# hztools/go-sdr

Hardware: AMD Instinct MI355X
Metric: Msamples/s: u8->c64->Shift->FIR-decimate chain @1 GPU; 4-ch Beamform @1/2/4 GPU (higher is better)
Workload: dtype u8 x int32 fixed-point taps (int8 MFMA digit planes, exact) -> c64(f32), NCO phase 64-bit fixed point

## Files before the change

go-sdr_amd/csrc/hz_firmm2.h:

```cpp
#pragma once
#include <type_traits>

#include "hz_firmm.h"
#include "hz_firmm2_plan.h"

namespace hz {
namespace mm2 {

using mm::v16i;
using mm::v4i;

using mm::find_le;
using mm::task_window;

struct KernArgs {
    const void *in;
    float2 *out;
    const float2 *hist;
    float2 *new_hist;
    const uint8_t *rhist;
    uint8_t *new_rhist;
    const float2 *taps;
    size_t n_in;
    Geom G;
// ... 33 lines not shown
        return make_float2(__fmaf_rn(v.x, cr, -(v.y * ci)), __fmaf_rn(v.x, ci, v.y * cr));
    };
#pragma unroll
    for (int b = 0; b < NB; b++) {
        double zc = cc0, zs = cs0;
#pragma unroll
        for (int q = 0; q < 4; q++) {
            y[4 * b + q] = mul32(y[4 * b + q], zc, zs);
            if (q < 3) {
                const double nc = __fma_rn(zc, e_c, -(zs * e_s)), ns = __fma_rn(zc, e_s, zs * e_c);
                zc = nc;
                zs = ns;
            }
        }
        if (b + 1 < NB) {
            const double nc = __fma_rn(cc0, b_c, -(cs0 * b_s)), ns = __fma_rn(cc0, b_s, cs0 * b_c);
            cc0 = nc;
            cs0 = ns;
        }
    }
}

typedef float v2f __attribute__((ext_vector_type(2)));
__device__ __forceinline__ v2f pk_turn(v2f cs0, v2f wxy, v2f wzw) {
    v2f t;
    asm("v_pk_mul_f32 %0, %1, %2 op_sel:[1,1] op_sel_hi:[1,0] neg_lo:[0,1]" : "=v"(t) : "v"(cs0), "v"(wzw));
    asm("v_pk_fma_f32 %0, %1, %2, %0 op_sel_hi:[0,1,1]" : "+v"(t) : "v"(cs0), "v"(wzw));
    asm("v_pk_fma_f32 %0, %1, %2, %0 op_sel:[1,1,0] op_sel_hi:[1,0,1] neg_lo:[0,1,0]" : "+v"(t) : "v"(cs0), "v"(wxy));
    asm("v_pk_fma_f32 %0, %1, %2, %0 op_sel_hi:[0,1,1]" : "+v"(t) : "v"(cs0), "v"(wxy));
    return t;
}
__device__ __forceinline__ v2f pk_cmul(v2f y, v2f f) {
    v2f u, r;
    asm("v_pk_mul_f32 %0, %1, %2 op_sel:[1,1] op_sel_hi:[1,0] neg_lo:[0,1]" : "=v"(u) : "v"(y), "v"(f));
    asm("v_pk_fma_f32 %0, %1, %2, %3 op_sel_hi:[0,1,1]" : "=v"(r) : "v"(y), "v"(f), "v"(u));
    return r;
}

template <int FMT, int D, int NG = 0, int EXP = 0, int UG = 0>
__global__ __launch_bounds__(kThreads) void fir_mm2_kernel(
    const void *__restrict__ in, float2 *__restrict__ out, const float2 *__restrict__ hist,
    float2 *__restrict__ new_hist, const uint8_t *__restrict__ rhist, uint8_t *__restrict__ new_rhist,
    const float2 *__restrict__ taps, size_t n_in, Geom G, Plan L, EwProgram P, Fix F, Batch B,
    unsigned long long *stamps = nullptr) {
    extern __shared__ __attribute__((aligned(16))) uint8_t mm_lds[];
    constexpr int TB = tile_bytes(D), PPT = TB / 16, GS = PPT / 2, NB = blocks_for(D);
    constexpr int kPassOut = pass_out(D);
    constexpr bool STRAIGHT = NG > 0 && UG == 0;
    constexpr int KU = NG > 0 ? ((pass_tiles(D) - 1 + NG) * PPT + 63) / 64 : kU;
    constexpr bool kWhole = NG > 0 && ((pass_tiles(D) - 1 + NG) * PPT) % 64 == 0;
    constexpr bool kPlane = STRAIGHT && D == 8 && (EXP & (1 << 29)) != 0;
    static_assert(!kPlane || (EXP & (256 | 524288 | (1 << 23) | (1 << 27) | (1 << 28))) == 0, "not with the pair loop's experiments");
    static_assert(!kPlane || plane_form(D, NG * GS, 0), "the host sizes the LDS by plane_form");
    constexpr int TS = tile_stride(D, kPlane);
    const int tid = threadIdx.x, wave = __builtin_amdgcn_readfirstlane(tid >> 6), l = tid & 63;
    const int wb = blockIdx.x;
    const int n = l & 31, h = l >> 5;
    const size_t tab_lds = table_lds(G.ne), slot_sz = slot_bytes(D, G.ks, kPlane);
    uint8_t *const tabp = mm_lds;
    unsigned *const ctr = reinterpret_cast<unsigned *>(mm_lds + 2 * tab_lds);
    uint8_t *const slot = mm_lds + 2 * tab_lds + kCtlBytes + (size_t)wave * slot_sz;
    const int64_t n_bytes = 2 * (int64_t)n_in;
    const uint8_t *src = (const uint8_t *)in;
    const int pieces = (int)(image_bytes(D, G.ks) / 16);
    const int nbuf = B.nbuf;
    const uint32_t rcp = B.rcp;
    const int64_t nb = (int64_t)B.nb;
    auto buf_of = [&](uint32_t pass) -> int { return nbuf > 1 ? (int)__umulhi(pass, rcp) : 0; };
    auto vin_of = [&](int j) -> uint64_t { return j == 0 ? (uint64_t)(uintptr_t)src : B.vin[j]; };
    auto vout_of = [&](int j) -> uint64_t { return j == 0 ? (uint64_t)(uintptr_t)out : B.vout[j]; };
    typedef const v4i __attribute__((address_space(1))) *gload_p;
    constexpr bool kStampShare = kPlane && (EXP & 64) != 0;
    static_assert(!kStampShare || (8 * 16 * 8 * kWaves <= 8192 && 2 * slot_bytes(D, NG * GS, true) >= task_bytes(D, 1025)), "the shared areas fit");
    constexpr int kStampRows = (EXP & (1 << 24)) != 0 ? 16 : 4;
    int stamp_pass = 0;
    [[maybe_unused]] unsigned long long *const lstamp =
        reinterpret_cast<unsigned long long *>(mm_lds + lds_bytes(D, G.ks, G.ne, G.ntaps, kPlane) - (kStampShare ? task_bytes(D, G.ntaps) : 0)) +
        (size_t)wave * (8 * kStampRows);
    if constexpr ((EXP & 64) != 0) {
        for (int i = l; i < 8 * kStampRows; i += 64) lstamp[i] = 0;
    }
    auto stamp = [&](int k) {
        if constexpr ((EXP & 64) != 0) {
            if (l == 0 && stamp_pass < kStampRows)
                lstamp[(k == 0 || k == 7 || (k >= 8 && k < 16) ? 0 : stamp_pass) * 8 + (k & 7)] = __builtin_amdgcn_s_memrealtime();
        }
    };
    stamp(0);
    [[maybe_unused]] unsigned long long clk0 = 0, rt0 = 0;
    if constexpr ((EXP & 64) != 0) clk0 = __builtin_amdgcn_s_memtime(), rt0 = __builtin_amdgcn_s_memrealtime();
    if constexpr ((EXP & 32) != 0) __builtin_amdgcn_s_setprio(1);
    const Run run0 = L.run[0];
    {
        const uint64_t a0 = (uint64_t)(uintptr_t)in, a1 = (uint64_t)n_in, a2 = (uint64_t)(uintptr_t)run0.tab;
        asm volatile("" ::"s"(a0), "s"(a1), "s"(a2), "s"(G.w0), "s"(G.ks), "s"(G.ne), "s"(G.e0), "s"(G.ntaps), "s"(G.off), "s"(L.n),
                     "s"(L.n_pass), "s"(L.grid), "s"(L.n_task), "s"(L.pass_first[0]), "s"(L.pass_end[0]), "s"(L.pass_first[1]),
                     "s"(L.pass_end[1]), "s"(run0.m_lo), "s"(run0.m_hi), "s"(nbuf), "s"(rcp), "s"(nb));
    }

    const uint32_t NP = (uint32_t)L.n_pass;
    const uint32_t per = NP / (uint32_t)L.grid, rem = NP - per * (uint32_t)L.grid;
    const uint32_t pb0 = (uint32_t)wb * per + min((uint32_t)wb, rem), pb1 = pb0 + per + ((uint32_t)wb < rem ? 1u : 0u);

    auto pass_p0 = [&](uint32_t pass) { return 2 * ((int64_t)D * ((int64_t)pass * kPassOut) - G.w0); };
    auto inside = [&](uint32_t pass) {
        const int64_t p0 = pass_p0(pass), lo = (int64_t)buf_of(pass) * nb;
        return p0 >= lo && p0 + 16 * (int64_t)pieces <= lo + nb;
    };
    auto issue = [&](v4i(&x)[KU], uint32_t pass) {
        const gload_p p = (gload_p)(vin_of(buf_of(pass)) + (uint64_t)pass_p0(pass));
        const gload_p pl = p + l;
#pragma unroll
        for (int u = 0; u < KU; u++) {
            x[u] = v4i{0, 0, 0, 0};
            if constexpr ((EXP & 1) != 0) continue;
            if constexpr (kWhole) x[u] = __builtin_nontemporal_load(pl + 64 * u);
            else x[u] = __builtin_nontemporal_load(p + min(l + u * 64, pieces - 1));
        }
    };
    v4i x[KU];
    bool pre_issued = false;
    if (wave < kWaves / 2) {
        const uint32_t p = pb0 + (uint32_t)wave;
        if (pb0 >= (uint32_t)L.pass_first[0] && p < min(pb1, (uint32_t)L.pass_end[0]) && inside(p)) {
            issue(x, p);
            pre_issued = true;
        }
    }
    using RWT = typename Raw<FMT>::t;
    uint32_t fix_m0 = 0;
    int fix_cnt = 0;
    auto task_xs = [&](const Geom &G) {
        return reinterpret_cast<float2 *>(mm_lds + 2 * table_lds(G.ne) + kCtlBytes + (kStampShare ? 0 : (size_t)kWaves * slot_bytes(D, G.ks, kPlane)));
    };
    auto tasks_front_cold = [&](int round, const void *in, const float2 *hist, float2 *new_hist, const uint8_t *rhist, uint8_t *new_rhist,
                                const float2 *taps, size_t n_in, const Geom &G, const Plan &L, const EwProgram &P, const Fix &F, const Batch &B) {
        auto vbase = [&](int64_t pu) -> const RWT * {
            const void *sb = in;
            for (int i = 1; i < B.nbuf; i++)
                if (2 * pu >= (int64_t)i * (int64_t)B.nb) sb = (const void *)(uintptr_t)B.vin[i];
            return (const RWT *)sb;
        };
        float2 *const xs = task_xs(G);
        float2 *const tl = xs + (G.ntaps + D * (kFixOut - 1));
        const int ftask = (L.grid - 1 - wb) + round * L.grid;
        if (ftask < L.n_task) {
            const int ct = tid;
            const int k = find_le(F.task_first, F.n, ftask);
            fix_m0 = F.m_a[k] + (uint32_t)(ftask - F.task_first[k]) * kFixOut;
            fix_cnt = (int)min((uint32_t)kFixOut, F.m_b[k] - fix_m0);
            if (round == 0)
                for (int q = ct; q < G.ntaps; q += 256) tl[q] = taps[q];
            const int64_t p_lo = (int64_t)D * fix_m0 - (G.ntaps - 1);
            const int n_s = G.ntaps + D * (fix_cnt - 1);
            const NcoWin tw = task_window(P, p_lo, p_lo + n_s - 1);
#pragma unroll 1
            for (int i0 = ct; i0 < n_s; i0 += 5 * 256) {
                constexpr int W = 5;
                float2 v[W];
#pragma unroll
                for (int u = 0; u < W; u++) {
                    const int64_t pu = p_lo + i0 + u * 256;
                    v[u] = Raw<FMT>::cvt((i0 + u * 256 < n_s && pu >= 0) ? vbase(pu)[pu] : RWT{});
                }
                ew_apply_n<W, 2>(P, v, (uint64_t)(p_lo + i0), tw, (uint64_t)256);
#pragma unroll
                for (int u = 0; u < W; u++) {
                    const int idx = i0 + u * 256;
                    const int64_t pu = p_lo + idx;
                    if (idx < n_s)
                        xs[idx] = pu >= 0 ? v[u] : ((hist && pu + (int64_t)G.off >= 0) ? hist[pu + (int64_t)G.off] : make_float2(0.f, 0.f));
                }
            }
        }
    };
    auto history_tasks_cold = [&](const void *in0, const float2 *hist, float2 *new_hist, const uint8_t *rhist, uint8_t *new_rhist, size_t n_in,
                                  const Geom &G, const Plan &L, const EwProgram &P, const Batch &B) {
        const void *const in = B.nbuf > 1 ? (const void *)(uintptr_t)B.vin[B.nbuf - 1] : in0;
        const int n_hist_tasks = new_hist ? (int)((G.off + kHistPer - 1) / kHistPer) : 0;
        for (int j = wb + L.grid * wave; j < n_hist_tasks; j += (kWaves / 2) * L.grid) {
            const unsigned idx = (unsigned)j * kHistPer + l;
            const int64_t h_lo = (int64_t)n_in - (int64_t)G.off + (int64_t)j * kHistPer;
            const NcoWin tw = task_window(P, h_lo, h_lo + kHistPer - 1);
            if (idx < G.off) {
                const int64_t p = (int64_t)n_in - (int64_t)G.off + idx;
                new_hist[idx] = mm::ordered_sample<FMT, 2>(in, P, p, hist, G.off, tw);
// ... 13 lines not shown
    auto tasks_front = [&](int round) {
        if (wave >= kWaves / 2) return;
        if ((L.grid - 1 - wb) + round * L.grid >= L.n_task) return;
        if constexpr ((EXP & 4096) != 0) {
            tasks_front_cold(round, in, hist, new_hist, rhist, new_rhist, taps, n_in, G, L, P, F, B);
        } else {
            HZ_COLD_ARGS;
            tasks_front_cold(round, in, hist, new_hist, rhist, new_rhist, taps, n_in, G, L, P, F, B);
        }
    };
    auto tasks_back_cold = [&](float2 *out0, const Geom &G, const Batch &B) {
        float2 *const xs = task_xs(G);
        float2 *const tl = xs + (G.ntaps + D * (kFixOut - 1));
        const int ct = tid;
        const int o = ct >> 4, sl = ct & 15;
        double ar = 0.0, ai = 0.0;
        if (o < fix_cnt) {
            const float2 *xo = xs + D * o + (G.ntaps - 1);
#pragma unroll 4
            for (int kk = sl; kk < G.ntaps; kk += 16) {
                const float2 hk = tl[kk], x = xo[-kk];
                const double xr = x.x, xi = x.y, hr = hk.x, hi = hk.y;
                ar = __fma_rn(xr, hr, ar);
                ar = __fma_rn(-xi, hi, ar);
                ai = __fma_rn(xr, hi, ai);
                ai = __fma_rn(xi, hr, ai);
            }
        }
#pragma unroll
        for (int d = 1; d < 16; d <<= 1) {
            ar += __shfl_xor(ar, d);
            ai += __shfl_xor(ai, d);
        }
        if (o < fix_cnt && sl == 0) {
            float2 *ob = out0;
            for (int i = 1; i < B.nbuf; i++)
                if (fix_m0 + o >= (uint32_t)i * B.out_each) ob = (float2 *)(uintptr_t)B.vout[i];
            ob[fix_m0 + o] = make_float2((float)ar, (float)ai);
        }
        fix_cnt = 0;
    };
    auto tasks_back = [&]() {
        if (wave >= kWaves / 2 || fix_cnt == 0) return;
        if constexpr ((EXP & 4096) != 0) {
            tasks_back_cold(out, G, B);
        } else {
            HZ_COLD_ARGS;
            tasks_back_cold(out, G, B);
        }
    };
    stamp(9);
    auto put = [&](int q, v4i v) {
        if constexpr (FMT == HZSDR_FMT_U8) v ^= (int)0x80808080;
        *reinterpret_cast<v4i *>(slot + TS * (q / PPT) + 16 * (q % PPT)) = v;
    };
    auto vm_clear = [&]() {
        if constexpr ((EXP & 128) == 0) __builtin_amdgcn_s_waitcnt(0x0F70);
    };
    auto land = [&](v4i(&x)[KU], bool flipped = false) {
        uint8_t *lp = slot + TS * (l / PPT) + 16 * (l % PPT);
        if constexpr (FMT == HZSDR_FMT_U8 && STRAIGHT && (EXP & 262144) != 0 && (EXP & (1 << 25)) != 0 && (EXP & 32768) == 0) {
            if (!flipped) {
#pragma unroll
                for (int u = 0; u < KU; u++) {
                    x[u] ^= (int)0x80808080;
                    asm volatile("" : "+v"(x[u]));
                }
            }
        }
#pragma unroll
        for (int u = 0; u < KU; u++)
            if (kWhole || l + u * 64 < pieces) {
                if constexpr (FMT == HZSDR_FMT_U8 && (EXP & 32768) == 0) {
                    if constexpr (STRAIGHT && (EXP & 262144) != 0 && (EXP & (1 << 25)) != 0) {
                    } else if constexpr (STRAIGHT && (EXP & 262144) != 0) {
                        if (!flipped) x[u] ^= (int)0x80808080;
                    } else {
                        x[u] ^= (int)0x80808080;
                    }
                }
                *reinterpret_cast<v4i *>(lp + u * (64 / PPT) * TS) = x[u];
            }
        if constexpr (FMT == HZSDR_FMT_U8 && (EXP & 32768) != 0) {
#pragma unroll
            for (int u = 0; u < KU; u++)
                if (kWhole || l + u * 64 < pieces) {
                    unsigned long long *q8 = reinterpret_cast<unsigned long long *>(lp + u * (64 / PPT) * TS);
                    (void)__hip_atomic_fetch_xor(q8, 0x8080808080808080ull, __ATOMIC_RELAXED, __HIP_MEMORY_SCOPE_WAVEFRONT);
                    (void)__hip_atomic_fetch_xor(q8 + 1, 0x8080808080808080ull, __ATOMIC_RELAXED, __HIP_MEMORY_SCOPE_WAVEFRONT);
                }
        }
        __builtin_amdgcn_fence(__ATOMIC_RELEASE, "wavefront");
        __builtin_amdgcn_wave_barrier();
    };
    auto land_edge_cold = [&](uint32_t pass, const uint8_t *src, const uint8_t *rhist, int64_t n_bytes, const Geom &G, const Plan &L, const Batch &B) {
        const int64_t p0 = 2 * ((int64_t)D * ((int64_t)pass * kPassOut) - G.w0);
        const int pieces = (int)(image_bytes(D, G.ks) / 16);
#pragma unroll 1
        for (int q = l; q < pieces; q += 64) {
            const int64_t p = p0 + (int64_t)q * 16;
            v4i v{0, 0, 0, 0};
            if (p >= 0 && p + 16 <= n_bytes) {
                uint64_t sb = (uint64_t)(uintptr_t)src;
                for (int i = 1; i < B.nbuf; i++)
                    if (p >= (int64_t)i * (int64_t)B.nb) sb = B.vin[i];
                v = *(const v4i __attribute__((address_space(1))) *)(sb + (uint64_t)p);
            } else if (p < 0 && L.cont && p + 2 * (int64_t)G.off >= 0) {
                v = *reinterpret_cast<const v4i *>(rhist + (p + 2 * (int64_t)G.off));
            } else if (p + 16 > 0 && p < n_bytes) {
                uint64_t w0 = 0, w1 = 0;
#pragma unroll 1
                for (int e = 0; e < 16; e++)
                    if (p + e >= 0 && p + e < n_bytes) {
                        const uint64_t bb = src[p + e];
                        if (e < 8) w0 |= bb << (8 * e);
                        else w1 |= bb << (8 * (e - 8));
                    }
                v = v4i{(int)(uint32_t)w0, (int)(uint32_t)(w0 >> 32), (int)(uint32_t)w1, (int)(uint32_t)(w1 >> 32)};
            }
            put(q, v);
        }
        __builtin_amdgcn_fence(__ATOMIC_RELEASE, "wavefront");
        __builtin_amdgcn_wave_barrier();
    };
    auto land_edge = [&](uint32_t pass) {
        if constexpr ((EXP & 4096) != 0) {
            land_edge_cold(pass, src, rhist, n_bytes, G, L, B);
        } else {
            HZ_COLD_ARGS;
            land_edge_cold(pass, (const uint8_t *)in, rhist, 2 * (int64_t)n_in, G, L, B);
        }
    };

    const int i_row = 4 * ((n >> 2) & 1) + (n >> 3);
    const int a_base = 64 * ((D / 8) * i_row - h + G.e0) + 16 * (n & 3);
    const int f_stride = G.ne * 64;
    const int groups = NG > 0 ? NG : G.ks / GS;

    [[maybe_unused]] auto plane_loop = [&](v4i(&pa)[4][4], int tab_off) {
        constexpr int KP = NG * GS / 2;
        constexpr int NE = 2 * (2 * KP + 4) + (D / 8) * (kT - 1) + 1;
        const int r16 = l & 15, kq = l >> 4;
        int a_off = plane_a_offset(NE, G.e0, 0, KP - 1, r16, kq) + tab_off;
        asm volatile("" : "+v"(a_off));
        const uint8_t *ap = tabp + a_off;
        const uint8_t *bp = slot + TS * r16 + 16 * kq;
        uint64_t p0_mask = (G.p0_hi >= 64 ? ~0ull : (1ull << G.p0_hi) - 1) & ~((1ull << G.p0_lo) - 1);
        v4i a[2][4], b[2][4];
        auto load = [&](auto tc) {
            constexpr int t = decltype(tc)::value, r = t & 1;
#pragma unroll
            for (int u = 0; u < 8; u++) {
                const int p = u == 0 ? 1 : u < 5 ? -1 : u == 7 ? 0 : u - 3, j = u - 1;
                if (p >= 0) a[r][p] = *reinterpret_cast<const v4i *>(ap + 32 * NE * p + 128 * (KP - 1 - t));
                else b[r][j] = *reinterpret_cast<const v4i *>(bp + TS * (16 * j + t / 2) + 64 * (t & 1));
            }
        };
        constexpr bool kFirstC0 = (EXP & 65536) != 0;
        if constexpr (!kFirstC0) {
#pragma unroll
            for (int p = 1; p < 4; p++)
#pragma unroll
                for (int j = 0; j < 4; j++) pa[p][j] = v4i{0, 0, 0, 0};
        }
#pragma unroll
        for (int j = 0; j < 4; j++) pa[0][j] = v4i{0, 0, 0, 0};
        load(std::integral_constant<int, 0>{});
        auto pair = [&](auto self, auto tc) {
            constexpr int t = decltype(tc)::value, r = t & 1;
            if constexpr (t < KP) {
                if constexpr (t + 1 < KP) load(std::integral_constant<int, t + 1>{});
#pragma unroll
                for (int p = 1; p < 4; p++)
#pragma unroll
                    for (int j = 0; j < 4; j++) {
                        if constexpr (kFirstC0 && t == 0)
                            asm volatile("v_mfma_i32_16x16x64_i8 %0, %1, %2, 0" : "=&v"(pa[p][j]) : "v"(a[r][p]), "v"(b[r][j]));
                        else
                            pa[p][j] = __builtin_amdgcn_mfma_i32_16x16x64_i8(a[r][p], b[r][j], pa[p][j], 0, 0, 0);
                    }
                if constexpr (FMT == HZSDR_FMT_U8 && (EXP & 262144) != 0) {
                    constexpr int kFlipFirst = KP - 1 - (KU + 3) / 4;
                    if constexpr (t == kFlipFirst) __builtin_amdgcn_s_waitcnt(0x0F70);
                    if constexpr (t >= kFlipFirst && 4 * (t - kFlipFirst) < KU) {
#pragma unroll
                        for (int u = 4 * (t - kFlipFirst); u < KU && u < 4 * (t - kFlipFirst) + 4; u++) {
                            x[u] ^= (int)0x80808080;
                            asm volatile("" : "+v"(x[u]));
                        }
                    }
                }
#pragma unroll
                for (int q = 0; q < 8; q++) {
                    __builtin_amdgcn_sched_group_barrier(0x008, 1, 0);
                    if constexpr (t + 1 < KP) __builtin_amdgcn_sched_group_barrier(0x100, 1, 0);
                }
                __builtin_amdgcn_sched_group_barrier(0x008, 4, 0);
                __builtin_amdgcn_sched_barrier(0);
                asm volatile("" : "+s"(p0_mask));
                if ((p0_mask >> t) & 1) {
#pragma unroll
                    for (int j = 0; j < 4; j++) pa[0][j] = __builtin_amdgcn_mfma_i32_16x16x64_i8(a[r][0], b[r][j], pa[0][j], 0, 0, 0);
                }
                __builtin_amdgcn_sched_barrier(0);
                self(self, std::integral_constant<int, t + 1>{});
            }
        };
        pair(pair, std::integral_constant<int, 0>{});
    };

    bool first_seg = true, first_stamp = true;
    const double k3 = __hiloint2double((1023 - G.shift) << 20, 0), k2 = k3 * 256.0, k1 = k3 * 65536.0, k0 = k3 * 16777216.0;
    auto planes = [&](const v16i(&acc)[2][NB], float2(&y)[NB][4], double dcr, double dci) {
#pragma unroll
        for (int b = 0; b < NB; b++)
#pragma unroll
            for (int aa = 0; aa < 4; aa++) {
                float c2[2];
#pragma unroll
                for (int pt = 0; pt < 2; pt++) {
                    const int q = 4 * aa + 2 * pt;
                    if constexpr ((EXP & (1 << 27)) != 0) {
                        const int hi = (int)(((unsigned)acc[0][b][q] << 8) + (unsigned)acc[0][b][q + 1]);
                        float v = __fmaf_rn((float)acc[1][b][q + 1], (float)k3, (float)(pt ? dci : dcr));
                        v = __fmaf_rn((float)acc[1][b][q], (float)k2, v);
                        c2[pt] = __fmaf_rn((float)hi, (float)k1, v);
                        continue;
                    }
                    double v = __fma_rn((double)acc[1][b][q + 1], k3, pt ? dci : dcr);
                    v = __fma_rn((double)acc[1][b][q], k2, v);
                    if constexpr ((EXP & 16384) != 0) {
                        const int hi = (int)(((unsigned)acc[0][b][q] << 8) + (unsigned)acc[0][b][q + 1]);
                        v = __fma_rn((double)hi, k1, v);
                    } else {
                        v = __fma_rn((double)acc[0][b][q + 1], k1, v);
                        v = __fma_rn((double)acc[0][b][q], k0, v);
                    }
                    c2[pt] = (float)v;
                }
                y[b][aa] = make_float2(c2[0], c2[1]);
            }
    };
    auto planes16 = [&](const v4i(&pa)[4][4], float2(&y)[NB][4], double dcr, double dci) {
        float z[4][2][2];
#pragma unroll
        for (int j = 0; j < 4; j++)
#pragma unroll
            for (int k = 0; k < 4; k++) {
                const int pt = k & 1;
                double v = __fma_rn((double)pa[3][j][k], k3, pt ? dci : dcr);
                v = __fma_rn((double)pa[2][j][k], k2, v);
                if constexpr ((EXP & 16384) != 0) {
                    const int hi = (int)(((unsigned)pa[0][j][k] << 8) + (unsigned)pa[1][j][k]);
                    v = __fma_rn((double)hi, k1, v);
                } else {
                    v = __fma_rn((double)pa[1][j][k], k1, v);
                    v = __fma_rn((double)pa[0][j][k], k0, v);
                }
                z[j][k >> 1][pt] = (float)v;
            }
#pragma unroll
        for (int b = 0; b < NB; b++)
#pragma unroll
            for (int a2 = 0; a2 < 2; a2++) {
                float w[2][2];
#pragma unroll
                for (int pt = 0; pt < 2; pt++) {
                    const auto sw = __builtin_amdgcn_permlane16_swap(__float_as_uint(z[2 * b][a2][pt]), __float_as_uint(z[2 * b + 1][a2][pt]), false, false);
                    w[0][pt] = __uint_as_float(sw[0]);
                    w[1][pt] = __uint_as_float(sw[1]);
                }
                y[b][a2] = make_float2(w[0][0], w[0][1]);
                y[b][2 + a2] = make_float2(w[1][0], w[1][1]);
            }
    };
    auto program = [&](float2(&y)[NB][4], uint32_t mb, uint64_t phi_r, uint64_t dphi, int seg, const float4 *wtab) {
        auto other_stage = [&](int oi, int seg, const EwProgram &P) {
            const EwOp &o = P.op[oi];
            if (o.kind == EW_SCALE) {
#pragma unroll
                for (int b = 0; b < NB; b++)
#pragma unroll
                    for (int q = 0; q < 4; q++) {
                        float gx = __fmul_rn(y[b][q].x, o.a), gy = __fmul_rn(y[b][q].y, o.a);
                        asm volatile("" : "+v"(gx), "+v"(gy));
                        y[b][q] = make_float2(gx, gy);
                    }
            } else if (o.kind == EW_ROTATE) {
#pragma unroll
                for (int b = 0; b < NB; b++)
#pragma unroll
                    for (int q = 0; q < 4; q++) y[b][q] = go_cmul(y[b][q], make_float2(o.a, o.b));
            } else {
                const double step = P.segs.step[seg];
                const int64_t dj = (int64_t)((uint64_t)D * mb) - (int64_t)P.segs.first[seg];
                const double ts0 = __fma_rn((double)dj, step, P.segs.t0[seg]);
                float2 t[4 * NB];
#pragma unroll
                for (int b = 0; b < NB; b++)
#pragma unroll
                    for (int q = 0; q < 4; q++) t[4 * b + q] = y[b][q];
                other_shift_stage<D, NB>(t, o.tau_shift, step, ts0, l);
#pragma unroll
                for (int b = 0; b < NB; b++)
#pragma unroll
                    for (int q = 0; q < 4; q++) y[b][q] = t[4 * b + q];
            }
        };
        auto shift_stage = [&]() {
                const uint64_t ph0 = phi_r + (uint64_t)D * mb * dphi;
                float s0, c0;
                if constexpr ((EXP & (1 << 20)) != 0) s0 = __uint_as_float((uint32_t)(ph0 >> 40)), c0 = 1.0f;
                else sincos_turns32((uint32_t)(ph0 >> 32), s0, c0);
                [[maybe_unused]] float4 wpin[4 * NB];
                [[maybe_unused]] float4 chk_w = make_float4(0.f, 0.f, 0.f, 0.f);
                [[maybe_unused]] float chk_cs = 0.f, chk_sn = 0.f;
                if constexpr ((EXP & 512) != 0) {
#pragma unroll
                    for (int i = 1; i < 4 * NB; i++) wpin[i] = wtab[i];
                    asm volatile("s_waitcnt lgkmcnt(0)\n s_nop 7" ::: "memory");
#pragma unroll
                    for (int i = 1; i < 4 * NB; i++) asm volatile("" : "+v"(wpin[i].x), "+v"(wpin[i].y), "+v"(wpin[i].z), "+v"(wpin[i].w));
                }
                if constexpr ((EXP & 8192) != 0) {
                    const v2f cs0{c0, s0};
#pragma unroll
                    for (int b = 0; b < NB; b++)
// ... 350 lines not shown
                    }
                }
            }
            stamp(2);
            [[maybe_unused]] int cs_e1 = 0, cs_e2 = 0, cs_l1 = 0, cs_l2 = 0;
            [[maybe_unused]] auto csum = [&](int &s1, int &s2) {
#pragma unroll
                for (int f = 0; f < 2; f++)
#pragma unroll
                    for (int b = 0; b < NB; b++) asm volatile("" : "+v"(acc[f][b]));
                s1 = 0, s2 = 0;
#pragma unroll
                for (int f = 0; f < 2; f++)
#pragma unroll
                    for (int b = 0; b < NB; b++)
#pragma unroll
                        for (int q = 0; q < 16; q++) s1 += acc[f][b][q], s2 += (1 + q + 16 * (b + NB * f)) * acc[f][b][q];
                asm volatile("" : "+v"(s1), "+v"(s2));
            };
            if constexpr ((EXP & 256) != 0) csum(cs_e1, cs_e2);
            if (in_next) land(x, active && (EXP & 2) == 0);
            else if (has_next) land_edge(pass_of(nxt));
            vm_clear();
            stamp(3);
            if constexpr ((EXP & 256) != 0) {
                csum(cs_l1, cs_l2);
                v4i *ref = reinterpret_cast<v4i *>((uintptr_t)stamps[1]);
                const size_t ci = (size_t)pass_of(cur) * 64 + l;
                if (active) {
                    if (stamps[0] == 0) {
                        ref[ci] = v4i{cs_e1, cs_e2, cs_l1, cs_l2};
                    } else {
                        const v4i r = ref[ci];
                        if (r[0] != cs_e1 || r[1] != cs_e2 || r[2] != cs_l1 || r[3] != cs_l2) {
                            const unsigned long long slot_r = atomicAdd(&stamps[2], 1ull);
                            if (slot_r < 4000) {
                                unsigned long long *rec = stamps + 8 + 8 * slot_r;
                                rec[0] = (unsigned long long)pass_of(cur) | ((unsigned long long)l << 32) | ((unsigned long long)wave << 40);
                                rec[1] = (unsigned long long)(unsigned)wb | ((unsigned long long)(unsigned)__builtin_amdgcn_s_getreg(4 | (31 << 11)) << 32);
                                rec[2] = (unsigned long long)(unsigned)cs_e1 | ((unsigned long long)(unsigned)cs_e2 << 32);
                                rec[3] = (unsigned long long)(unsigned)cs_l1 | ((unsigned long long)(unsigned)cs_l2 << 32);
                                rec[4] = (unsigned long long)(unsigned)r[0] | ((unsigned long long)(unsigned)r[1] << 32);
                                rec[5] = (unsigned long long)(unsigned)r[2] | ((unsigned long long)(unsigned)r[3] << 32);
                                rec[6] = __builtin_amdgcn_s_memrealtime();
                                rec[7] = (unsigned long long)(unsigned)__builtin_amdgcn_s_getreg(20 | (31 << 11));
                            }
                        }
                    }
                }
            }
            if (active) {
                const double *dc = reinterpret_cast<const double *>(tabp + tab_off + (size_t)G.ne * 128);
                float2 y[NB][4];
                if constexpr (kPlane) planes16(pacc, y, dc[0] * k3, dc[1] * k3);
                else planes(acc, y, dc[0] * k3, dc[1] * k3);
                if constexpr ((EXP & 64) != 0) {
#pragma unroll
                    for (int b = 0; b < NB; b++)
#pragma unroll
                        for (int q = 0; q < 4; q++) asm volatile("" : "+v"(y[b][q].x), "+v"(y[b][q].y));
                }
                stamp(4);
                const uint32_t mb = m_start + (uint32_t)n * kT + 4 * h;
                {
                    program(y, mb, phi_r, dphi, sel ? rv.seg : ru.seg, reinterpret_cast<const float4 *>(dc + 2));
                    stamp(5);
                    const uint64_t outp = vout_of(buf_of(pass_of(cur)));
                    if constexpr (kDefer) {
#pragma unroll
                        for (int b = 0; b < NB; b++)
#pragma unroll
                            for (int q = 0; q < 4; q++) yd[b][q] = y[b][q];
                        out_d = outp, mb_d = mb, lo_d = v_lo, hi_d = v_hi, have_d = true;
                        if (!has_next) flush_deferred();
                    } else {
#pragma unroll
                        for (int b = 0; b < NB; b++) store_block(outp, y[b], mb + (uint32_t)(32 * kT) * b, v_lo, v_hi);
                    }
                }
            }
            stamp(6);
            if constexpr ((EXP & 32) != 0) __builtin_amdgcn_s_setprio(0);
            cur = nxt;
        }
        if (!b_here) break;
        ra = rb;
        slot_a ^= 1;
        a_done = true;
        if (!has_passes(ra + 1)) break;
    }
    history_tasks();
#pragma unroll 1
    for (int round = 0; (L.grid - 1 - wb) + round * L.grid < L.n_task; round++) {
        if (round > 0 || kStampShare) __syncthreads();
        tasks_front(round);
        __syncthreads();
        tasks_back();
    }
    stamp(7);
    if constexpr ((EXP & 64) != 0) {
        for (int i = l; i < 8 * kStampRows; i += 64) stamps[((size_t)wb * kWaves + wave) * (8 * kStampRows) + i] = lstamp[i];
        if (tid == 0) {
            unsigned long long *ck = stamps + (size_t)L.grid * kWaves * (8 * kStampRows) + 2 * (size_t)wb;
            ck[0] = __builtin_amdgcn_s_memtime() - clk0;
            ck[1] = __builtin_amdgcn_s_memrealtime() - rt0;
        }
    }
// ... 10 lines not shown
```

go-sdr_amd/csrc/hz_firmm2.hip:

```cpp
#if defined(HZSDR_NO_PK_F32) && defined(__HIP_DEVICE_COMPILE__)
#pragma clang attribute push(__attribute__((target("no-packed-fp32-ops"))), apply_to = function)
#endif

#include <stdlib.h>

#include <algorithm>

#include "hz_firmm2.h"

namespace hz {
namespace mm2 {

template <class K, class... A>
static int launch(K kernel, dim3 grid, size_t lds, hipStream_t stream, A... args) {
    if (lds > 48 * 1024) HZ_TRY(raise_dynamic_lds((const void *)kernel));
    hipLaunchKernelGGL(kernel, grid, dim3(kThreads), lds, stream, args...);
    return hipGetLastError() == hipSuccess ? HZSDR_OK : HZSDR_ERR_HIP;
}

constexpr int kLibExp = 8192 | 16384 | 65536 | 131072 | 262144 | (1 << 22) | (1 << 25) | (1 << 26) | (1 << 29);
constexpr int kPairExp = kLibExp & ~(1 << 29);

template <int FMT>
static int launch_fmt(hipStream_t stream, int num_cus, unsigned D, const void *in, float2 *out, const float2 *hist,
                      float2 *new_hist, const uint8_t *rhist, uint8_t *new_rhist, const float2 *taps, size_t n, const Geom &g,
                      Plan L, const EwProgram &P, const Fix &F, const Batch &B, int rolled) {
    if (!factor_ok(D)) return HZSDR_ERR_INVALID_ARGUMENT;
    const bool plane = plane_form((int)D, g.ks, rolled);
    const size_t lds = lds_bytes((int)D, g.ks, g.ne, g.ntaps, plane);
    if (D == 16) {
        const int grid16 = std::max(1, L.grid);
        unsigned long long *no_stamps16 = nullptr;
        if (g.ks == 9 * 8 && rolled == 0)
            return launch(fir_mm2_kernel<FMT, 16, 9, kLibExp>, dim3(grid16), lds, stream, in, out, hist, new_hist, rhist, new_rhist, taps, n, g, L, P, F, B, no_stamps16);
        return launch(fir_mm2_kernel<FMT, 16, 0, kLibExp>, dim3(grid16), lds, stream, in, out, hist, new_hist, rhist, new_rhist, taps, n, g, L, P, F, B, no_stamps16);
    }
    const int grid = std::max(1, L.grid);
    (void)num_cus;
    unsigned long long *no_stamps = nullptr;
    if (plane)
        return launch(fir_mm2_kernel<FMT, 8, 17, kLibExp>, dim3(grid), lds, stream, in, out, hist, new_hist, rhist, new_rhist, taps, n, g, L, P, F, B, no_stamps);
    if (g.ks == 17 * 4 && rolled == 8)
        return launch(fir_mm2_kernel<FMT, 8, 17, kPairExp>, dim3(grid), lds, stream, in, out, hist, new_hist, rhist, new_rhist, taps, n, g, L, P, F, B, no_stamps);
    if (g.ks == 17 * 4 && rolled == 1)
        return launch(fir_mm2_kernel<FMT, 8, 17, kLibExp, 1>, dim3(grid), lds, stream, in, out, hist, new_hist, rhist, new_rhist, taps, n, g, L, P, F, B, no_stamps);
    if (g.ks == 17 * 4 && rolled == 2)
        return launch(fir_mm2_kernel<FMT, 8, 17, kLibExp, 2>, dim3(grid), lds, stream, in, out, hist, new_hist, rhist, new_rhist, taps, n, g, L, P, F, B, no_stamps);
    if (g.ks == 17 * 4 && rolled == 4)
        return launch(fir_mm2_kernel<FMT, 8, 17, kLibExp, 4>, dim3(grid), lds, stream, in, out, hist, new_hist, rhist, new_rhist, taps, n, g, L, P, F, B, no_stamps);
    return launch(fir_mm2_kernel<FMT, 8, 0, kLibExp>, dim3(grid), lds, stream, in, out, hist, new_hist, rhist, new_rhist, taps, n, g, L, P, F, B, no_stamps);
}

int launch_fir(hipStream_t stream, int num_cus, int fmt, unsigned D, const void *in, float2 *out, const float2 *hist,
               float2 *new_hist, const uint8_t *rhist, uint8_t *new_rhist, const float2 *taps, size_t n, const Geom &g,
               const Plan &L, const EwProgram &P, const Fix &F, const Batch &B, int loop_form) {
    if (fmt == HZSDR_FMT_U8)
        return launch_fmt<HZSDR_FMT_U8>(stream, num_cus, D, in, out, hist, new_hist, rhist, new_rhist, taps, n, g, L, P, F, B, loop_form);
    if (fmt == HZSDR_FMT_I8)
        return launch_fmt<HZSDR_FMT_I8>(stream, num_cus, D, in, out, hist, new_hist, rhist, new_rhist, taps, n, g, L, P, F, B, loop_form);
    return HZSDR_ERR_INVALID_ARGUMENT;
}

template <int FMT>
__global__ __launch_bounds__(64) void history_kernel(const void *__restrict__ in, float2 *__restrict__ new_hist, uint8_t *__restrict__ new_rhist,
                                                     size_t n_in, unsigned off, EwProgram P) {
    using RWT = typename Raw<FMT>::t;
    const unsigned idx = blockIdx.x * 64u + threadIdx.x;
    const int64_t h_lo = (int64_t)n_in - (int64_t)off + (int64_t)blockIdx.x * 64;
    const NcoWin tw = mm::task_window(P, h_lo, h_lo + 63);
    if (idx < off) {
        const int64_t p = (int64_t)n_in - (int64_t)off + idx;
        new_hist[idx] = mm::ordered_sample<FMT, 2>(in, P, p, nullptr, off, tw);
        reinterpret_cast<RWT *>(new_rhist)[idx] = ((const RWT *)in)[p];
    }
}

int launch_history(hipStream_t stream, int fmt, const void *in, float2 *new_hist, uint8_t *new_rhist, size_t n, unsigned off, const EwProgram &P) {
    if (n < off || off == 0) return HZSDR_ERR_INVALID_ARGUMENT;
    const dim3 grid((off + 63) / 64), block(64);
    if (fmt == HZSDR_FMT_U8) hipLaunchKernelGGL(history_kernel<HZSDR_FMT_U8>, grid, block, 0, stream, in, new_hist, new_rhist, n, off, P);
    else if (fmt == HZSDR_FMT_I8) hipLaunchKernelGGL(history_kernel<HZSDR_FMT_I8>, grid, block, 0, stream, in, new_hist, new_rhist, n, off, P);
    else return HZSDR_ERR_INVALID_ARGUMENT;
    return hipGetLastError() == hipSuccess ? HZSDR_OK : HZSDR_ERR_HIP;
}

}
}

#if defined(HZSDR_NO_PK_F32) && defined(__HIP_DEVICE_COMPILE__)
#pragma clang attribute pop
#endif
```

go-sdr_amd/csrc/hz_firmm2_plan.h:

```cpp
#pragma once
#include <math.h>
#include <stddef.h>
#include <stdint.h>
#include <string.h>

namespace hz {
namespace mm2 {

constexpr int kT = 8;
constexpr int kWaves = 8;
constexpr int kThreads = 64 * kWaves;
constexpr int kFixOut = 16;
constexpr int kHistPer = 64;
constexpr int kMaxRuns = 16;
constexpr int kMaxClockRuns = 32;
constexpr int kMaxFix = kMaxClockRuns + 2;
constexpr uint64_t kShortRun = 1280;
constexpr int kU = 12;

constexpr bool factor_ok(unsigned D) { return D == 8 || D == 16; }
constexpr int blocks_for(int D) { return D >= 16 ? 1 : 2; }
constexpr int tile_bytes(int D) { return 2 * D * kT; }
constexpr int pass_tiles(int D) { return 32 * blocks_for(D); }
constexpr int pass_out(int D) { return pass_tiles(D) * kT; }
constexpr size_t image_bytes(int D, int ks) { return (size_t)(pass_tiles(D) - 1) * tile_bytes(D) + 32 * (size_t)ks; }
constexpr int tile_stride(int D, bool plane = false) { return tile_bytes(D) + (plane ? 32 : 16); }
constexpr bool plane_form(int D, int ks, int loop_form) { return D == 8 && ks == 17 * 4 && loop_form == 0; }
constexpr size_t slot_bytes(int D, int ks, bool plane = false) {
    return ((image_bytes(D, ks) / tile_bytes(D) + 1) * tile_stride(D, plane) + 255) / 256 * 256;
}
constexpr size_t table_bytes(int ne) { return (size_t)ne * 128 + 16 + 128; }
constexpr size_t table_lds(int ne) { return (table_bytes(ne) + 255) / 256 * 256; }
constexpr size_t kCtlBytes = 512;
constexpr size_t task_bytes(int D, int ntaps) { return ((size_t)(2 * ntaps + D * (kFixOut - 1)) * 8 + 255) / 256 * 256; }
constexpr size_t lds_bytes(int D, int ks, int ne, int ntaps, bool plane = false) {
    return 2 * table_lds(ne) + kCtlBytes + kWaves * slot_bytes(D, ks, plane) + task_bytes(D, ntaps);
}

constexpr int plane_piece(int ne, int q) {
    return q >= 8 * ne ? q : ((2 * (q / (4 * ne)) + (q & 1)) * ne + (q % (4 * ne)) / 4) * 2 + ((q >> 1) & 1);
}
constexpr int plane_a_offset(int ne, int e0, int p, int t, int r16, int kq) {
    return 32 * ne * p + 32 * ((r16 >> 1) - kq - 4 * t + e0) + 16 * (r16 & 1);
}
constexpr int plane_b_offset(int ts, int j, int t, int r16, int kq) { return ts * (16 * j + t / 2 + r16) + 64 * (t & 1) + 16 * kq; }

struct Geom {
    int ntaps;
    int w0;
    int ks;
    int ne;
    int e0;
    int shift;
    unsigned off;
    int p0_lo, p0_hi;
};

struct Run {
    const void *tab;
    uint32_t m_lo, m_hi;
    int pass_first;
    int pass_end;
    uint64_t phi, dphi;
    uint64_t first;
    int seg;
    int pad[3];
};
static_assert(sizeof(Run) == 64, "one scalar-cache line per run");
struct Plan {
    int n;
    int n_pass;
    int cont;
    int shift_op;
    int n_task;
    int n_ops;
    float gain;
    int grid;
    int pass_first[kMaxRuns], pass_end[kMaxRuns];
    Run run[kMaxRuns];
};
struct Fix {
    int n;
    int n_task;
    uint32_t m_a[kMaxFix], m_b[kMaxFix];
    int task_first[kMaxFix];
};
constexpr int kMaxBatch = 8;
struct Batch {
    int nbuf;
// ... 228 lines not shown
```

Before: 700,500.

## Add register-reusing B-operand plane loop with LDS exchange for output transpose

Adds a new default D=8 plane loop variant that lays out the input image in the LDS slot with a new row layout (128-byte rows, padded every four). Across consecutive tap steps it rotates B-operand registers, so after the first two steps only one new B quad per step is read from LDS instead of four. It also replaces the plane reduction's output shuffle with a per-wave LDS exchange area for redistributing results. The intent is to cut LDS read traffic in the MFMA inner loop. The cost is a different slot size, extra exchange writes and wave barriers in the epilogue, and reworked scheduling hints.

```diff
diff --git a/go-sdr_amd/csrc/hz_firmm2.h b/go-sdr_amd/csrc/hz_firmm2.h
--- a/go-sdr_amd/csrc/hz_firmm2.h
+++ b/go-sdr_amd/csrc/hz_firmm2.h
@@ -109,11 +109,15 @@
     constexpr bool kPlane = STRAIGHT && D == 8 && (EXP & (1 << 29)) != 0;
     static_assert(!kPlane || (EXP & (256 | 524288 | (1 << 23) | (1 << 27) | (1 << 28))) == 0, "not with the pair loop's experiments");
     static_assert(!kPlane || plane_form(D, NG * GS, 0), "the host sizes the LDS by plane_form");
+    constexpr bool kReuse = kPlane && (EXP & (1 << 30)) != 0;
+    static_assert((EXP & (1 << 30)) == 0 || kPlane, "the re-using loop is a per-plane loop");
+    static_assert(!kReuse || ((EXP & 32768) == 0 && kXchgBytes == 2 * 64 * 16), "the landing by plain writes; two quads per lane and half in the exchange area");
     constexpr int TS = tile_stride(D, kPlane);
+    auto row_at = [](int r) { return kReuse ? reuse_row_offset(r) : TS * r; };
     const int tid = threadIdx.x, wave = __builtin_amdgcn_readfirstlane(tid >> 6), l = tid & 63;
     const int wb = blockIdx.x;
     const int n = l & 31, h = l >> 5;
-    const size_t tab_lds = table_lds(G.ne), slot_sz = slot_bytes(D, G.ks, kPlane);
+    const size_t tab_lds = table_lds(G.ne), slot_sz = form_slot_bytes(D, G.ks, kPlane, kReuse);
     uint8_t *const tabp = mm_lds;
     unsigned *const ctr = reinterpret_cast<unsigned *>(mm_lds + 2 * tab_lds);
     uint8_t *const slot = mm_lds + 2 * tab_lds + kCtlBytes + (size_t)wave * slot_sz;
@@ -128,11 +132,11 @@
     auto vout_of = [&](int j) -> uint64_t { return j == 0 ? (uint64_t)(uintptr_t)out : B.vout[j]; };
     typedef const v4i __attribute__((address_space(1))) *gload_p;
     constexpr bool kStampShare = kPlane && (EXP & 64) != 0;
-    static_assert(!kStampShare || (8 * 16 * 8 * kWaves <= 8192 && 2 * slot_bytes(D, NG * GS, true) >= task_bytes(D, 1025)), "the shared areas fit");
+    static_assert(!kStampShare || (8 * 16 * 8 * kWaves <= 8192 && 2 * form_slot_bytes(D, NG * GS, true, kReuse) >= task_bytes(D, 1025)), "the shared areas fit");
     constexpr int kStampRows = (EXP & (1 << 24)) != 0 ? 16 : 4;
     int stamp_pass = 0;
     [[maybe_unused]] unsigned long long *const lstamp =
-        reinterpret_cast<unsigned long long *>(mm_lds + lds_bytes(D, G.ks, G.ne, G.ntaps, kPlane) - (kStampShare ? task_bytes(D, G.ntaps) : 0)) +
+        reinterpret_cast<unsigned long long *>(mm_lds + form_lds_bytes(D, G.ks, G.ne, G.ntaps, kPlane, kReuse) - (kStampShare ? task_bytes(D, G.ntaps) : 0)) +
         (size_t)wave * (8 * kStampRows);
     if constexpr ((EXP & 64) != 0) {
         for (int i = l; i < 8 * kStampRows; i += 64) lstamp[i] = 0;
@@ -188,7 +192,7 @@
     uint32_t fix_m0 = 0;
     int fix_cnt = 0;
     auto task_xs = [&](const Geom &G) {
-        return reinterpret_cast<float2 *>(mm_lds + 2 * table_lds(G.ne) + kCtlBytes + (kStampShare ? 0 : (size_t)kWaves * slot_bytes(D, G.ks, kPlane)));
+        return reinterpret_cast<float2 *>(mm_lds + 2 * table_lds(G.ne) + kCtlBytes + (kStampShare ? 0 : (size_t)kWaves * form_slot_bytes(D, G.ks, kPlane, kReuse)));
     };
     auto tasks_front_cold = [&](int round, const void *in, const float2 *hist, float2 *new_hist, const uint8_t *rhist, uint8_t *new_rhist,
                                 const float2 *taps, size_t n_in, const Geom &G, const Plan &L, const EwProgram &P, const Fix &F, const Batch &B) {
@@ -308,13 +312,15 @@
     stamp(9);
     auto put = [&](int q, v4i v) {
         if constexpr (FMT == HZSDR_FMT_U8) v ^= (int)0x80808080;
-        *reinterpret_cast<v4i *>(slot + TS * (q / PPT) + 16 * (q % PPT)) = v;
+        *reinterpret_cast<v4i *>(slot + row_at(q / PPT) + 16 * (q % PPT)) = v;
     };
     auto vm_clear = [&]() {
         if constexpr ((EXP & 128) == 0) __builtin_amdgcn_s_waitcnt(0x0F70);
     };
     auto land = [&](v4i(&x)[KU], bool flipped = false) {
-        uint8_t *lp = slot + TS * (l / PPT) + 16 * (l % PPT);
+        uint8_t *lp = slot + row_at(l / PPT) + 16 * (l % PPT);
+        constexpr int kLandStep = kReuse ? reuse_row_offset(64 / PPT) : (64 / PPT) * TS;
+        static_assert(!kReuse || (64 / PPT) % 4 == 0, "whole groups of four rows");
         if constexpr (FMT == HZSDR_FMT_U8 && STRAIGHT && (EXP & 262144) != 0 && (EXP & (1 << 25)) != 0 && (EXP & 32768) == 0) {
             if (!flipped) {
 #pragma unroll
@@ -335,13 +341,13 @@
                         x[u] ^= (int)0x80808080;
                     }
                 }
-                *reinterpret_cast<v4i *>(lp + u * (64 / PPT) * TS) = x[u];
+                *reinterpret_cast<v4i *>(lp + u * kLandStep) = x[u];
             }
         if constexpr (FMT == HZSDR_FMT_U8 && (EXP & 32768) != 0) {
 #pragma unroll
             for (int u = 0; u < KU; u++)
                 if (kWhole || l + u * 64 < pieces) {
-                    unsigned long long *q8 = reinterpret_cast<unsigned long long *>(lp + u * (64 / PPT) * TS);
+                    unsigned long long *q8 = reinterpret_cast<unsigned long long *>(lp + u * kLandStep);
                     (void)__hip_atomic_fetch_xor(q8, 0x8080808080808080ull, __ATOMIC_RELAXED, __HIP_MEMORY_SCOPE_WAVEFRONT);
                     (void)__hip_atomic_fetch_xor(q8 + 1, 0x8080808080808080ull, __ATOMIC_RELAXED, __HIP_MEMORY_SCOPE_WAVEFRONT);
                 }
@@ -400,7 +406,7 @@
         int a_off = plane_a_offset(NE, G.e0, 0, KP - 1, r16, kq) + tab_off;
         asm volatile("" : "+v"(a_off));
         const uint8_t *ap = tabp + a_off;
-        const uint8_t *bp = slot + TS * r16 + 16 * kq;
+        const uint8_t *bp = slot + row_at(kReuse ? 4 * r16 : r16) + 16 * kq;
         uint64_t p0_mask = (G.p0_hi >= 64 ? ~0ull : (1ull << G.p0_hi) - 1) & ~((1ull << G.p0_lo) - 1);
         v4i a[2][4], b[2][4];
         auto load = [&](auto tc) {
@@ -409,9 +415,11 @@
             for (int u = 0; u < 8; u++) {
                 const int p = u == 0 ? 1 : u < 5 ? -1 : u == 7 ? 0 : u - 3, j = u - 1;
                 if (p >= 0) a[r][p] = *reinterpret_cast<const v4i *>(ap + 32 * NE * p + 128 * (KP - 1 - t));
-                else b[r][j] = *reinterpret_cast<const v4i *>(bp + TS * (16 * j + t / 2) + 64 * (t & 1));
+                else if constexpr (!kReuse) b[r][j] = *reinterpret_cast<const v4i *>(bp + TS * (16 * j + t / 2) + 64 * (t & 1));
+                else if (reuse_b_read(j, t)) b[r][reuse_b_reg(j, t)] = *reinterpret_cast<const v4i *>(bp + reuse_row_offset(j + t / 2) + 64 * (t & 1));
             }
         };
+        auto bsel = [](int j, int t) { return kReuse ? reuse_b_reg(j, t) : j; };
         constexpr bool kFirstC0 = (EXP & 65536) != 0;
         if constexpr (!kFirstC0) {
 #pragma unroll
@@ -431,9 +439,9 @@
 #pragma unroll
                     for (int j = 0; j < 4; j++) {
                         if constexpr (kFirstC0 && t == 0)
-                            asm volatile("v_mfma_i32_16x16x64_i8 %0, %1, %2, 0" : "=&v"(pa[p][j]) : "v"(a[r][p]), "v"(b[r][j]));
+                            asm volatile("v_mfma_i32_16x16x64_i8 %0, %1, %2, 0" : "=&v"(pa[p][j]) : "v"(a[r][p]), "v"(b[r][bsel(j, t)]));
                         else
-                            pa[p][j] = __builtin_amdgcn_mfma_i32_16x16x64_i8(a[r][p], b[r][j], pa[p][j], 0, 0, 0);
+                            pa[p][j] = __builtin_amdgcn_mfma_i32_16x16x64_i8(a[r][p], b[r][bsel(j, t)], pa[p][j], 0, 0, 0);
                     }
                 if constexpr (FMT == HZSDR_FMT_U8 && (EXP & 262144) != 0) {
                     constexpr int kFlipFirst = KP - 1 - (KU + 3) / 4;
@@ -446,17 +454,18 @@
                         }
                     }
                 }
-#pragma unroll
-                for (int q = 0; q < 8; q++) {
+                constexpr int kReads = kReuse && t + 1 >= 2 ? 5 : 8;
+#pragma unroll
+                for (int q = 0; q < kReads; q++) {
                     __builtin_amdgcn_sched_group_barrier(0x008, 1, 0);
                     if constexpr (t + 1 < KP) __builtin_amdgcn_sched_group_barrier(0x100, 1, 0);
                 }
-                __builtin_amdgcn_sched_group_barrier(0x008, 4, 0);
+                __builtin_amdgcn_sched_group_barrier(0x008, 12 - kReads, 0);
                 __builtin_amdgcn_sched_barrier(0);
                 asm volatile("" : "+s"(p0_mask));
                 if ((p0_mask >> t) & 1) {
 #pragma unroll
-                    for (int j = 0; j < 4; j++) pa[0][j] = __builtin_amdgcn_mfma_i32_16x16x64_i8(a[r][0], b[r][j], pa[0][j], 0, 0, 0);
+                    for (int j = 0; j < 4; j++) pa[0][j] = __builtin_amdgcn_mfma_i32_16x16x64_i8(a[r][0], b[r][bsel(j, t)], pa[0][j], 0, 0, 0);
                 }
                 __builtin_amdgcn_sched_barrier(0);
                 self(self, std::integral_constant<int, t + 1>{});
@@ -529,6 +538,49 @@
                 y[b][a2] = make_float2(w[0][0], w[0][1]);
                 y[b][2 + a2] = make_float2(w[1][0], w[1][1]);
             }
+    };
+    [[maybe_unused]] auto planes_xchg = [&](const v4i(&pa)[4][4], float2(&y)[NB][4], double dcr, double dci) {
+        typedef float v4f_ __attribute__((ext_vector_type(4)));
+        static_assert(!kReuse || NB == 2, "two halves of 32 tiles");
+        v4f_ z[4];
+#pragma unroll
+        for (int j = 0; j < 4; j++)
+#pragma unroll
+            for (int k = 0; k < 4; k++) {
+                const int pt = k & 1;
+                double v = __fma_rn((double)pa[3][j][k], k3, pt ? dci : dcr);
+                v = __fma_rn((double)pa[2][j][k], k2, v);
+                if constexpr ((EXP & 16384) != 0) {
+                    const int hi = (int)(((unsigned)pa[0][j][k] << 8) + (unsigned)pa[1][j][k]);
+                    v = __fma_rn((double)hi, k1, v);
+                } else {
+                    v = __fma_rn((double)pa[1][j][k], k1, v);
+                    v = __fma_rn((double)pa[0][j][k], k0, v);
+                }
+                z[j][k] = (float)v;
+            }
+        int lx = l;
+        asm volatile("" : "+v"(lx));
+        uint8_t *const xb = slot + reuse_image_bytes(D, NG * GS);
+        uint8_t *const we = xb + xchg_write_offset(lx, 0), *const wo = xb + xchg_write_offset(lx, 1);
+        const uint8_t *const rp = xb + xchg_read_offset(lx, 0);
+#pragma unroll
+        for (int b = 0; b < 2; b++) {
+            if (xchg_half(lx) == b) {
+#pragma unroll
+                for (int j = 0; j < 4; j++) *reinterpret_cast<v4f_ *>(((j & 1) ? wo : we) + 128 * (j >> 1)) = z[j];
+            }
+            __builtin_amdgcn_fence(__ATOMIC_RELEASE, "wavefront");
+            __builtin_amdgcn_wave_barrier();
+#pragma unroll
+            for (int q = 0; q < 2; q++) {
+                const v4f_ w = *reinterpret_cast<const v4f_ *>(rp + 1024 * q);
+                y[b][2 * q] = make_float2(w.x, w.y);
+                y[b][2 * q + 1] = make_float2(w.z, w.w);
+            }
+            __builtin_amdgcn_fence(__ATOMIC_ACQUIRE, "wavefront");
+            __builtin_amdgcn_wave_barrier();
+        }
     };
     auto program = [&](float2(&y)[NB][4], uint32_t mb, uint64_t phi_r, uint64_t dphi, int seg, const float4 *wtab) {
         auto other_stage = [&](int oi, int seg, const EwProgram &P) {
@@ -985,7 +1037,8 @@
             if (active) {
                 const double *dc = reinterpret_cast<const double *>(tabp + tab_off + (size_t)G.ne * 128);
                 float2 y[NB][4];
-                if constexpr (kPlane) planes16(pacc, y, dc[0] * k3, dc[1] * k3);
+                if constexpr (kReuse) planes_xchg(pacc, y, dc[0] * k3, dc[1] * k3);
+                else if constexpr (kPlane) planes16(pacc, y, dc[0] * k3, dc[1] * k3);
                 else planes(acc, y, dc[0] * k3, dc[1] * k3);
                 if constexpr ((EXP & 64) != 0) {
 #pragma unroll
diff --git a/go-sdr_amd/csrc/hz_firmm2.hip b/go-sdr_amd/csrc/hz_firmm2.hip
--- a/go-sdr_amd/csrc/hz_firmm2.hip
+++ b/go-sdr_amd/csrc/hz_firmm2.hip
@@ -20,14 +20,15 @@
 
 constexpr int kLibExp = 8192 | 16384 | 65536 | 131072 | 262144 | (1 << 22) | (1 << 25) | (1 << 26) | (1 << 29);
 constexpr int kPairExp = kLibExp & ~(1 << 29);
+constexpr int kReuseExp = kLibExp | (1 << 30);
 
 template <int FMT>
 static int launch_fmt(hipStream_t stream, int num_cus, unsigned D, const void *in, float2 *out, const float2 *hist,
                       float2 *new_hist, const uint8_t *rhist, uint8_t *new_rhist, const float2 *taps, size_t n, const Geom &g,
                       Plan L, const EwProgram &P, const Fix &F, const Batch &B, int rolled) {
     if (!factor_ok(D)) return HZSDR_ERR_INVALID_ARGUMENT;
-    const bool plane = plane_form((int)D, g.ks, rolled);
-    const size_t lds = lds_bytes((int)D, g.ks, g.ne, g.ntaps, plane);
+    const bool plane = plane_form((int)D, g.ks, rolled), reuse = reuse_form((int)D, g.ks, rolled);
+    const size_t lds = form_lds_bytes((int)D, g.ks, g.ne, g.ntaps, plane, reuse);
     if (D == 16) {
         const int grid16 = std::max(1, L.grid);
         unsigned long long *no_stamps16 = nullptr;
@@ -38,6 +39,8 @@
     const int grid = std::max(1, L.grid);
     (void)num_cus;
     unsigned long long *no_stamps = nullptr;
+    if (reuse)
+        return launch(fir_mm2_kernel<FMT, 8, 17, kReuseExp>, dim3(grid), lds, stream, in, out, hist, new_hist, rhist, new_rhist, taps, n, g, L, P, F, B, no_stamps);
     if (plane)
         return launch(fir_mm2_kernel<FMT, 8, 17, kLibExp>, dim3(grid), lds, stream, in, out, hist, new_hist, rhist, new_rhist, taps, n, g, L, P, F, B, no_stamps);
     if (g.ks == 17 * 4 && rolled == 8)
diff --git a/go-sdr_amd/csrc/hz_firmm2_plan.h b/go-sdr_amd/csrc/hz_firmm2_plan.h
--- a/go-sdr_amd/csrc/hz_firmm2_plan.h
+++ b/go-sdr_amd/csrc/hz_firmm2_plan.h
@@ -25,16 +25,43 @@
 constexpr int pass_out(int D) { return pass_tiles(D) * kT; }
 constexpr size_t image_bytes(int D, int ks) { return (size_t)(pass_tiles(D) - 1) * tile_bytes(D) + 32 * (size_t)ks; }
 constexpr int tile_stride(int D, bool plane = false) { return tile_bytes(D) + (plane ? 32 : 16); }
-constexpr bool plane_form(int D, int ks, int loop_form) { return D == 8 && ks == 17 * 4 && loop_form == 0; }
+constexpr int kLoopPair = 8, kLoopPlane = 9, kLoopReuse = 10;
+constexpr int kLoopDefault = kLoopReuse;
+constexpr bool plane_form(int D, int ks, int loop_form) {
+    return D == 8 && ks == 17 * 4 && (loop_form == 0 || loop_form == kLoopPlane || loop_form == kLoopReuse);
+}
+constexpr bool reuse_form(int D, int ks, int loop_form) {
+    return plane_form(D, ks, loop_form) && (loop_form == 0 ? kLoopDefault : loop_form) == kLoopReuse;
+}
 constexpr size_t slot_bytes(int D, int ks, bool plane = false) {
     return ((image_bytes(D, ks) / tile_bytes(D) + 1) * tile_stride(D, plane) + 255) / 256 * 256;
 }
+constexpr int reuse_row_offset(int row) { return 128 * row + 32 * (row >> 2); }
+constexpr int reuse_b_offset(int j, int t, int c, int kq) { return reuse_row_offset(4 * c + j + t / 2) + 64 * (t & 1) + 16 * kq; }
+constexpr int reuse_b_reg(int j, int t) { return (j + t / 2) & 3; }
+constexpr bool reuse_b_read(int j, int t) { return t < 2 || j == 3; }
+constexpr int kXchgBytes = 2048;
+constexpr size_t reuse_image_bytes(int D, int ks) {
+    return ((size_t)reuse_row_offset((int)(image_bytes(D, ks) / tile_bytes(D))) + 255) / 256 * 256;
+}
+constexpr size_t reuse_slot_bytes(int D, int ks) { return reuse_image_bytes(D, ks) + kXchgBytes; }
+constexpr int xchg_sigma(int d) {
+    return 32 * (d >> 5) + 16 * (d & 1) + 8 * ((d >> 1) & 1) + ((((d >> 2) & 7)) ^ (d & 1));
+}
+constexpr int xchg_dst_lane(int lane, int j) { return 32 * (lane >> 5) + 4 * (lane & 7) + j; }
+constexpr int xchg_half(int lane) { return (lane >> 3) & 1; }
+constexpr int xchg_write_offset(int lane, int j) { return 1024 * ((lane >> 4) & 1) + 16 * xchg_sigma(xchg_dst_lane(lane, j)); }
+constexpr int xchg_read_offset(int lane, int q) { return 1024 * q + 16 * xchg_sigma(lane); }
 constexpr size_t table_bytes(int ne) { return (size_t)ne * 128 + 16 + 128; }
 constexpr size_t table_lds(int ne) { return (table_bytes(ne) + 255) / 256 * 256; }
 constexpr size_t kCtlBytes = 512;
 constexpr size_t task_bytes(int D, int ntaps) { return ((size_t)(2 * ntaps + D * (kFixOut - 1)) * 8 + 255) / 256 * 256; }
 constexpr size_t lds_bytes(int D, int ks, int ne, int ntaps, bool plane = false) {
     return 2 * table_lds(ne) + kCtlBytes + kWaves * slot_bytes(D, ks, plane) + task_bytes(D, ntaps);
+}
+constexpr size_t form_slot_bytes(int D, int ks, bool plane, bool reuse) { return reuse ? reuse_slot_bytes(D, ks) : slot_bytes(D, ks, plane); }
+constexpr size_t form_lds_bytes(int D, int ks, int ne, int ntaps, bool plane, bool reuse) {
+    return 2 * table_lds(ne) + kCtlBytes + kWaves * form_slot_bytes(D, ks, plane, reuse) + task_bytes(D, ntaps);
 }
 
 constexpr int plane_piece(int ne, int q) {
```

Measured after the change: 709,400 (median of 6 runs). +1.3%, better.
